# cloneofsimo/vqgan-training

Measured on AMD Instinct MI355X. Metric: images/sec full train step (enc+dec+LPIPS+disc+bwd), 256x256 f=8, higher is better.
Workload: dtype mixed like the reference: encoder+LPIPS+discriminator fp16 operands (TF32's 10-bit mantissa) / fp32 accumulate, decoder bf16

## Files before the change

### vqgan-training_amd/csrc/conv_small.hip

```cpp
#include "vq_common.h"

struct SmallConvParams {
  VqConvDesc d;
  const vq_bf16* x;
  const vq_bf16* w;
  const float* bias;
  const vq_bf16* relu_mask;
  vq_bf16* y;
  int M, HoWo, Kp;
  float alpha;
  const float* alpha_dev;
};

template <int DT, int FC>
__global__ __launch_bounds__(256) void conv3x3_c8_kernel(const SmallConvParams p) {
  const int lane = threadIdx.x & 63;
  const int fr = lane & 31, fh = lane >> 5;
  const int wave_global = blockIdx.x * 4 + (threadIdx.x >> 6);
  const int nwaves = gridDim.x * 4;

  s16x8 wf[FC][5];
#pragma unroll
  for (int a = 0; a < FC; ++a)
#pragma unroll
    for (int kk = 0; kk < 5; ++kk) {
      int row = a * 32 + fr;
      if (row >= p.d.Cout) row = p.d.Cout - 1;
      wf[a][kk] = *(const s16x8*)(p.w + (int64_t)row * p.Kp + kk * 16 + fh * 8);
    }
  typedef Store<DT> St;
  const float alpha = p.alpha_dev ? p.alpha * *p.alpha_dev : p.alpha;
  constexpr int CP = FC * 32, SPR = CP / 8;
  __shared__ __attribute__((aligned(16))) vq_bf16 slabs[4 * 32 * CP];
  vq_bf16* slab = slabs + (threadIdx.x >> 6) * 32 * CP;
  float bv[FC][4][4];
#pragma unroll
  for (int a = 0; a < FC; ++a)
#pragma unroll
    for (int q = 0; q < 4; ++q)
#pragma unroll
      for (int e = 0; e < 4; ++e) {
        const int co = a * 32 + q * 8 + fh * 4 + e;
        bv[a][q][e] = (p.bias && co < p.d.Cout_w) ? p.bias[co] : 0.f;
      }
  const int ngroups = (p.M + 31) >> 5;
  for (int g = wave_global; g < ngroups; g += nwaves) {
    const int m = g * 32 + fr;
    const bool live = m < p.M;
    const int mm = live ? m : p.M - 1;
    const int n = mm / p.HoWo, rem = mm - n * p.HoWo;
    const int oy = rem / p.d.Wo, ox = rem - oy * p.d.Wo;
    s16x8 bf[5];
#pragma unroll
    for (int kk = 0; kk < 5; ++kk) {
      const int tap = 2 * kk + fh;
      const int r = tap / 3, s = tap - r * 3;
      const int iy = oy + r - 1, ix = ox + s - 1;
      const bool ok = live && tap < 9 && (unsigned)iy < (unsigned)p.d.H && (unsigned)ix < (unsigned)p.d.W;
      s16x8 z;
#pragma unroll
      for (int e = 0; e < 8; ++e) z[e] = 0;
      bf[kk] = ok ? *(const s16x8*)(p.x + ((int64_t)(n * p.d.H + iy) * p.d.W + ix) * 8) : z;
    }
    f32x16 acc[FC];
#pragma unroll
    for (int a = 0; a < FC; ++a)
#pragma unroll
      for (int e = 0; e < 16; ++e) acc[a][e] = 0.f;
#pragma unroll
    for (int kk = 0; kk < 5; ++kk)
#pragma unroll
      for (int a = 0; a < FC; ++a) acc[a] = mfma16<DT>(wf[a][kk], bf[kk], acc[a]);
#pragma unroll
    for (int a = 0; a < FC; ++a)
#pragma unroll
      for (int q = 0; q < 4; ++q) {
        const int co = a * 32 + q * 8 + fh * 4;
        float v[4];
#pragma unroll
        for (int e = 0; e < 4; ++e) {
          v[e] = acc[a][q * 4 + e] * alpha + bv[a][q][e];
          if (p.d.relu) v[e] = v[e] > 0.f ? v[e] : 0.f;
        }
        St::store4(slab, fr * CP + ((((co >> 3) + fr) % SPR) << 3) + (co & 4), v);
      }
    vq_wave_sync();
    const int64_t m0 = (int64_t)g * 32;
#pragma unroll
    for (int it = 0; it < (32 * SPR) / 64; ++it) {
      const int i = it * 64 + lane, p_l = i / SPR, sl = i % SPR;
      if (m0 + p_l >= p.M || sl * 8 >= p.d.Cout) continue;
      float v[8];
      St::load8(slab, p_l * CP + (((sl + p_l) % SPR) << 3), v);
      const int64_t off = (m0 + p_l) * p.d.Cout + sl * 8;
      if (p.relu_mask) {
        float mv[8];
        St::load8(p.relu_mask, off, mv);
#pragma unroll
        for (int e = 0; e < 8; ++e) v[e] = mv[e] > 0.f ? v[e] : 0.f;
      }
      St::store8(p.y, off, v);
    }
    vq_wave_sync();
  }
}

bool vq_conv_c8_shape(const VqConvDesc* d) {
  return d->subpix == 0 && (d->dtype == VQ_BF16 || d->dtype == VQ_F16) && d->split == 1 && d->Cin == 8 && d->R == 3 && d->S == 3 && d->stride == 1 && d->dil_in == 1 &&
         d->up == 1 && d->pad_t == 1 && d->pad_l == 1 && d->Cout <= 128 && d->Ho == d->H && d->Wo == d->W;
}
int vq_launch_conv_c8(const VqConvDesc* d, const void* x, const void* w_packed, const float* bias, const void* residual,
                      const void* relu_mask, void* y, float alpha, const float* alpha_dev, hipStream_t stream) {
  if (!vq_conv_c8_shape(d) || residual != nullptr) return 1;
  SmallConvParams p;
  p.d = *d; p.x = (const vq_bf16*)x; p.w = (const vq_bf16*)w_packed; p.bias = bias; p.relu_mask = (const vq_bf16*)relu_mask;
  p.y = (vq_bf16*)y;
  p.M = d->N * d->Ho * d->Wo; p.HoWo = d->Ho * d->Wo;
  p.Kp = vq_round_up(9 * 8, 64);
  p.alpha = alpha; p.alpha_dev = alpha_dev;
  const int ngroups = (p.M + 31) / 32;
  int blocks = (ngroups + 3) / 4;
  if (blocks > 2048) blocks = 2048;
  const int fc = (d->Cout + 31) / 32;
#define VQ_C8(DTv) do { \
    if (fc == 1) hipLaunchKernelGGL((conv3x3_c8_kernel<DTv, 1>), dim3(blocks), dim3(256), 0, stream, p); \
    else if (fc == 2) hipLaunchKernelGGL((conv3x3_c8_kernel<DTv, 2>), dim3(blocks), dim3(256), 0, stream, p); \
    else if (fc == 3) hipLaunchKernelGGL((conv3x3_c8_kernel<DTv, 3>), dim3(blocks), dim3(256), 0, stream, p); \
    else hipLaunchKernelGGL((conv3x3_c8_kernel<DTv, 4>), dim3(blocks), dim3(256), 0, stream, p); } while (0)
  if (d->dtype == VQ_F16) VQ_C8(VQ_F16); else VQ_C8(VQ_BF16);
#undef VQ_C8
  VQ_CHECK_LAUNCH("vq_conv2d_fwd(c8)");
  return VQ_OK;
}

template <int FC>
__global__ __launch_bounds__(256) void conv3x3_c8_x2_kernel(const SmallConvParams p) {
  typedef Store<VQ_F16X2> St;
  const int lane = threadIdx.x & 63, wave = threadIdx.x >> 6;
  const int fr = lane & 31, fh = lane >> 5;
  const int wave_global = blockIdx.x * 4 + wave, nwaves = gridDim.x * 4;
  __shared__ __attribute__((aligned(16))) float slabs[4 * 32 * 32];
  float* slab = slabs + wave * 32 * 32;
  const float alpha = p.alpha_dev ? p.alpha * *p.alpha_dev : p.alpha;
  const int ngroups = (p.M + 31) >> 5, nitems = ngroups * FC;
  int a_cur = -1;
  s16x8 wh[5], wl[5];
  float bv[4][4];
  for (int t = wave_global; t < nitems; t += nwaves) {
    const int g = t / FC, a = t - g * FC;
    if (a != a_cur) {
      a_cur = a;
      int row = a * 32 + fr;
      if (row >= p.d.Cout) row = p.d.Cout - 1;
#pragma unroll
      for (int kk = 0; kk < 5; ++kk) {
        const vq_bf16* src = p.w + (int64_t)row * p.Kp + (2 * kk + fh) * 16;
        wh[kk] = *(const s16x8*)src;
        wl[kk] = *(const s16x8*)(src + 8);
      }
#pragma unroll
      for (int q = 0; q < 4; ++q)
#pragma unroll
        for (int e = 0; e < 4; ++e) {
          const int co = a * 32 + q * 8 + fh * 4 + e;
          bv[q][e] = (p.bias && co < p.d.Cout_w) ? p.bias[co] : 0.f;
        }
    }
    const int m = g * 32 + fr;
    const bool live = m < p.M;
    const int mm = live ? m : p.M - 1;
    const int n = mm / p.HoWo, rem = mm - n * p.HoWo;
    const int oy = rem / p.d.Wo, ox = rem - oy * p.d.Wo;
    s16x8 bh[5], bl[5];
#pragma unroll
    for (int kk = 0; kk < 5; ++kk) {
      const int tap = 2 * kk + fh;
      const int r = tap / 3, sx = tap - r * 3;
      const int iy = oy + r - 1, ix = ox + sx - 1;
      const bool ok = live && tap < 9 && (unsigned)iy < (unsigned)p.d.H && (unsigned)ix < (unsigned)p.d.W;
      s16x8 z;
#pragma unroll
      for (int e = 0; e < 8; ++e) z[e] = 0;
      const vq_bf16* src = p.x + ((int64_t)(n * p.d.H + iy) * p.d.W + ix) * 16;
      bh[kk] = ok ? *(const s16x8*)src : z;
      bl[kk] = ok ? *(const s16x8*)(src + 8) : z;
    }
    f32x16 acc;
#pragma unroll
    for (int e = 0; e < 16; ++e) acc[e] = 0.f;
#pragma unroll
    for (int kk = 0; kk < 5; ++kk) {
      acc = mfma_32x32x16_f16(wh[kk], bl[kk], acc);
      acc = mfma_32x32x16_f16(wl[kk], bh[kk], acc);
      acc = mfma_32x32x16_f16(wh[kk], bh[kk], acc);
    }
#pragma unroll
    for (int q = 0; q < 4; ++q) {
      vq_f4 v;
      float t4[4];
#pragma unroll
      for (int e = 0; e < 4; ++e) {
        t4[e] = acc[q * 4 + e] * alpha + bv[q][e];
        if (p.d.relu) t4[e] = t4[e] > 0.f ? t4[e] : 0.f;
      }
      v.x = t4[0]; v.y = t4[1]; v.z = t4[2]; v.w = t4[3];
      *(vq_f4*)(slab + fr * 32 + (((q * 2 + fh) ^ (fr & 7)) << 2)) = v;
    }
    vq_wave_sync();
    const int64_t m0 = (int64_t)g * 32;
#pragma unroll
    for (int it = 0; it < 2; ++it) {
      const int i = it * 64 + lane, p_l = i >> 2, sl = i & 3;
      const int co = a * 32 + sl * 8;
      const vq_f4 lo4 = *(const vq_f4*)(slab + p_l * 32 + (((2 * sl) ^ (p_l & 7)) << 2));
      const vq_f4 hi4 = *(const vq_f4*)(slab + p_l * 32 + (((2 * sl + 1) ^ (p_l & 7)) << 2));
      if (m0 + p_l >= p.M || co >= p.d.Cout) continue;
      float v[8] = {lo4.x, lo4.y, lo4.z, lo4.w, hi4.x, hi4.y, hi4.z, hi4.w};
      const int64_t off = (m0 + p_l) * p.d.Cout + co;
      if (p.relu_mask) {
        float mv[8];
        St::load8(p.relu_mask, off, mv);
#pragma unroll
        for (int e = 0; e < 8; ++e) v[e] = mv[e] > 0.f ? v[e] : 0.f;
      }
      St::store8(p.y, off, v);
    }
    vq_wave_sync();
  }
}
bool vq_conv_c8_x2_shape(const VqConvDesc* d) {
  return d->dtype == VQ_F16X2 && d->subpix == 0 && d->split == 1 && d->Cin == 16 && d->R == 3 && d->S == 3 && d->stride == 1 && d->dil_in == 1 &&
         d->up == 1 && d->pad_t == 1 && d->pad_l == 1 && d->Cout <= 128 && d->Ho == d->H && d->Wo == d->W;
}
int vq_launch_conv_c8_x2(const VqConvDesc* d, const void* x, const void* w_packed, const float* bias, const void* residual,
                         const void* relu_mask, void* y, float alpha, const float* alpha_dev, hipStream_t stream) {
  if (!vq_conv_c8_x2_shape(d) || residual != nullptr) return 1;
  SmallConvParams p;
  p.d = *d; p.x = (const vq_bf16*)x; p.w = (const vq_bf16*)w_packed; p.bias = bias; p.relu_mask = (const vq_bf16*)relu_mask;
  p.y = (vq_bf16*)y;
  p.M = d->N * d->Ho * d->Wo; p.HoWo = d->Ho * d->Wo;
  p.Kp = vq_round_up(9 * 16, 64);
  p.alpha = alpha; p.alpha_dev = alpha_dev;
  const int fc = (d->Cout + 31) / 32;
  const int nitems = ((p.M + 31) / 32) * fc;
  int blocks = (nitems + 3) / 4;
  if (blocks > 2048) blocks = 2048;
  blocks = (blocks + 2) / 3 * 3;
  if (fc == 1) hipLaunchKernelGGL((conv3x3_c8_x2_kernel<1>), dim3(blocks), dim3(256), 0, stream, p);
  else if (fc == 2) hipLaunchKernelGGL((conv3x3_c8_x2_kernel<2>), dim3(blocks), dim3(256), 0, stream, p);
  else if (fc == 3) hipLaunchKernelGGL((conv3x3_c8_x2_kernel<3>), dim3(blocks), dim3(256), 0, stream, p);
  else hipLaunchKernelGGL((conv3x3_c8_x2_kernel<4>), dim3(blocks), dim3(256), 0, stream, p);
  VQ_CHECK_LAUNCH("vq_conv2d_fwd(c8, VQ_F16X2)");
  return VQ_OK;
}

struct SmallWgradParams {
  const vq_bf16* narrow;
  const vq_bf16* wide;
  float* part;
  int H, W, C;
  int M, runs_per_block, nruns;
  int nstride, noff;
};

template <int DT, int BT>
__global__ __launch_bounds__(256) void wgrad_c8_kernel(const SmallWgradParams p) {
  constexpr int RB = BT * 2, SPR = RB / 16, RPP = 1024 / RB, NPC = (64 / RPP) / 4;
  constexpr int XROW = 72 * 8;
  __shared__ __attribute__((aligned(16))) vq_bf16 lds[2 * 3 * XROW + 64 + 2 * 64 * BT];
  vq_bf16* zs = lds + 2 * 3 * XROW;
  auto xs_of = [&](int b) -> vq_bf16* { return lds + b * 3 * XROW; };
  auto ys_of = [&](int b) -> vq_bf16* { return lds + 2 * 3 * XROW + 64 + b * 64 * BT; };
  auto seg_key = [](int row) -> int { return RB >= 256 ? (row & 3) : ((row >> 1) & 1); };

  const int tid = threadIdx.x, lane = tid & 63, wave = tid >> 6;
  const int W = p.W, H = p.H;
  constexpr int NCF = BT / 32;
  const int my_cf = wave;
  f32x16 acc[3];
#pragma unroll
  for (int a = 0; a < 3; ++a)
#pragma unroll
    for (int e = 0; e < 16; ++e) acc[a][e] = 0.f;

  if (tid < 32) ((unsigned*)zs)[tid] = (tid == 30) ? (unsigned)One16<DT>::BITS : 0u;
  const int gg = lane >> 4, tl = lane & 15;
  int a_off[3];
  bool a_zero[3];
#pragma unroll
  for (int f = 0; f < 3; ++f) {
    const int tap = 4 * f + 2 * (gg & 1) + ((tl & 3) >> 1);
    a_zero[f] = tap >= 9;
    const int r = tap / 3, s = tap - r * 3;
    a_off[f] = a_zero[f] ? ((tap == 9 && (tl & 1) == 0) ? 60 : 0) : (r * XROW + (8 * (gg >> 1) + (tl >> 2) + s) * 8 + (tl & 1) * 4);
  }
  const int b_row = 8 * (gg >> 1) + (tl >> 2);
  const int b_col = (gg & 1) * 16 + (tl & 3) * 4;

  const int lrow = lane / SPR, lp = lane % SPR;
  const int ct0 = (int)blockIdx.y * BT;
  const int run0 = blockIdx.x * p.runs_per_block;
  int nhere = p.nruns - run0;
  if (nhere > p.runs_per_block) nhere = p.runs_per_block;

  auto stage_wide = [&](int run, int b) {
    const int m0 = run * 64;
    vq_bf16* ys = ys_of(b);
#pragma unroll
    for (int i = 0; i < NPC; ++i) {
      const int row = (wave * NPC + i) * RPP + lrow;
      const int seg = (lp >> 2) ^ seg_key(row);
      const int lsl = ((seg << 2) | (lp & 3)) << 3;
      glds16(p.wide + (int64_t)(m0 + row) * p.C + ct0 + lsl, ys + (wave * NPC + i) * RPP * BT);
    }
  };
  auto load_narrow = [&](int run) -> vq_u4 {
    vq_u4 v; v.x = v.y = v.z = v.w = 0u;
    if (tid < 3 * 66) {
      const int m0 = run * 64;
      const int n = m0 / (H * W), rem = m0 - n * H * W;
      const int oy = rem / W, ox0 = rem - oy * W;
      const int r = tid / 66, j = tid - r * 66;
      const int iy = oy + r - 1, ix = ox0 - 1 + j;
      if ((unsigned)iy < (unsigned)H && (unsigned)ix < (unsigned)W)
        v = *(const vq_u4*)(p.narrow + ((int64_t)(n * H + iy) * W + ix) * p.nstride + p.noff);
    }
    return v;
  };
  auto store_narrow = [&](int b, vq_u4 v) {
    if (tid < 3 * 66) {
      const int r = tid / 66, j = tid - r * 66;
      *(vq_u4*)(xs_of(b) + r * XROW + j * 8) = v;
    }
  };

  if (nhere > 0) {
    stage_wide(run0, 0);
    store_narrow(0, load_narrow(run0));
  }
  for (int rr = 0; rr < nhere; ++rr) {
    const int b = rr & 1;
    __syncthreads();
    const bool more = rr + 1 < nhere;
    vq_u4 nv; nv.x = nv.y = nv.z = nv.w = 0u;
    if (more) {
      stage_wide(run0 + rr + 1, b ^ 1);
      nv = load_narrow(run0 + rr + 1);
    }
    if (my_cf < NCF) {
      const vq_bf16* xs = xs_of(b);
      const char* yb = (const char*)ys_of(b);
#pragma unroll
      for (int kk = 0; kk < 4; ++kk) {
        const int c = my_cf * 32 + b_col;
        const int seg = (c * 2) >> 6, within = (c * 2) & 63;
        const int r0 = kk * 16 + b_row, r1 = r0 + 4;
        s16x4 lo4 = lds_read_tr16_b64((const short*)(yb + r0 * RB + ((seg ^ seg_key(r0)) << 6) + within));
        s16x4 hi4 = lds_read_tr16_b64((const short*)(yb + r1 * RB + ((seg ^ seg_key(r1)) << 6) + within));
        s16x8 bfr;
        bfr[0] = lo4[0]; bfr[1] = lo4[1]; bfr[2] = lo4[2]; bfr[3] = lo4[3];
        bfr[4] = hi4[0]; bfr[5] = hi4[1]; bfr[6] = hi4[2]; bfr[7] = hi4[3];
#pragma unroll
        for (int f = 0; f < 3; ++f) {
          const vq_bf16* base = a_zero[f] ? zs + a_off[f] : xs + a_off[f] + kk * 16 * 8;
          const int step = a_zero[f] ? 0 : 4 * 8;
          s16x4 al = lds_read_tr16_b64((const short*)base);
          s16x4 ah = lds_read_tr16_b64((const short*)(base + step));
          s16x8 af;
          af[0] = al[0]; af[1] = al[1]; af[2] = al[2]; af[3] = al[3];
          af[4] = ah[0]; af[5] = ah[1]; af[6] = ah[2]; af[7] = ah[3];
          acc[f] = mfma16<DT>(af, bfr, acc[f]);
        }
      }
    }
    if (more) store_narrow(b ^ 1, nv);
  }
  if (my_cf < NCF) {
    float* out = p.part + (int64_t)blockIdx.x * 96 * p.C;
    const int fr = lane & 31, fh = lane >> 5;
    const int c = ct0 + my_cf * 32 + fr;
#pragma unroll
    for (int f = 0; f < 3; ++f)
#pragma unroll
      for (int e = 0; e < 16; ++e) {
        const int i = f * 32 + (e & 3) + 8 * (e >> 2) + 4 * fh;
        out[(int64_t)i * p.C + c] = acc[f][e];
      }
  }
}

__global__ void wgrad_c8_reduce_kernel(const float* __restrict__ part, int nblk, int C, int Cout_w, int Cin_w,
                                       int swapped, int accumulate, float alpha, float* __restrict__ dw, float* __restrict__ dbias) {
  const int total = Cout_w * Cin_w * 9, total_b = total + (dbias ? Cout_w : 0);
  const int t = blockIdx.x * blockDim.x + threadIdx.x;
  const int i = t >> 3, sub = t & 7;
  const bool live = i < total_b, is_bias = i >= total;
  const int ii = (live && !is_bias) ? i : 0;
  const int tap = ii % 9, ci = (ii / 9) % Cin_w, co = is_bias ? (live ? i - total : 0) : ii / (9 * Cin_w);
  const int row = is_bias ? 72 : (swapped ? (8 - tap) * 8 + co : tap * 8 + ci), col = (swapped && !is_bias) ? ci : co;
  float s = 0.f;
  for (int b = sub; b < nblk; b += 8) s += part[((int64_t)b * 96 + row) * C + col];
  s += __shfl_xor(s, 1); s += __shfl_xor(s, 2); s += __shfl_xor(s, 4);
  s *= alpha;
  if (live && sub == 0) {
    float* dst = is_bias ? dbias + co : dw + ((int64_t)co * Cin_w + ci) * 9 + tap;
    *dst = accumulate ? (*dst + s) : s;
  }
}

static int c8_wgrad_blocks(const VqConvDesc* d) {
  const int nruns = d->N * d->Ho * d->Wo / 64;
  return nruns < 512 ? nruns : 512;
}
static bool c8_common(const VqConvDesc* d) {
  return (d->dtype == VQ_BF16 || d->dtype == VQ_F16) && d->split == 1 && d->R == 3 && d->S == 3 && d->stride == 1 && d->dil_in == 1 && d->up == 1 &&
         d->pad_t == 1 && d->pad_l == 1 && d->Ho == d->H && d->Wo == d->W && d->Wo % 64 == 0;
}
static bool c8_wide_ok(int c) { return c == 64 || (c % 128 == 0 && c >= 128 && c <= 1024); }
static bool c8_swapped(const VqConvDesc* d) { return d->Cout == 8 && c8_wide_ok(d->Cin); }
bool vq_wgrad_c8_eligible(const VqConvDesc* d) {
  return c8_common(d) && ((d->Cin == 8 && c8_wide_ok(d->Cout)) || c8_swapped(d));
}
size_t vq_wgrad_c8_workspace(const VqConvDesc* d) {
  return (size_t)c8_wgrad_blocks(d) * 96 * (c8_swapped(d) ? d->Cin : d->Cout) * sizeof(float);
}

static int c8_wgrad_grid(const VqConvDesc* d, int C, SmallWgradParams& p, dim3& grid) {
  p.H = d->H; p.W = d->W; p.C = C;
  p.M = d->N * d->Ho * d->Wo;
  p.nruns = p.M / 64;
  const int nblk = c8_wgrad_blocks(d);
  p.runs_per_block = (p.nruns + nblk - 1) / nblk;
  const int used = (p.nruns + p.runs_per_block - 1) / p.runs_per_block;
  grid = dim3(used, C >= 128 ? C / 128 : 1);
  return used;
}
#define WGRAD_C8_ROWS(X) X(VQ_F16, 128) X(VQ_F16, 64) X(VQ_BF16, 128) X(VQ_BF16, 64)
static void launch_wgrad_c8_pass(int dtype, const SmallWgradParams& p, dim3 grid, hipStream_t stream) {
  const int dt = dtype == VQ_F16 ? VQ_F16 : VQ_BF16, bt = vq_wgrad_c8_tile(p.C);
#define X(DT, BT) if (dt == DT && bt == BT) hipLaunchKernelGGL((wgrad_c8_kernel<DT, BT>), grid, dim3(256), 0, stream, p);
  WGRAD_C8_ROWS(X)
#undef X
}

int vq_launch_wgrad_c8(const VqConvDesc* d, const void* x, const void* dy, float* dw, float* dbias, int* dbias_done,
                       int accumulate, float alpha, void* workspace, hipStream_t stream) {
  const bool sw = c8_swapped(d);
  SmallWgradParams p;
  p.narrow = (const vq_bf16*)(sw ? dy : x); p.wide = (const vq_bf16*)(sw ? x : dy); p.part = (float*)workspace;
  p.nstride = 8; p.noff = 0;
  dim3 grid;
  const int used = c8_wgrad_grid(d, sw ? d->Cin : d->Cout, p, grid);
  launch_wgrad_c8_pass(d->dtype, p, grid, stream);
  VQ_CHECK_LAUNCH("vq_conv2d_wgrad(c8)");
  float* db = sw ? nullptr : dbias;
  *dbias_done = db != nullptr;
  const int total = d->Cout_w * d->Cin_w * 9 + (db ? d->Cout_w : 0);
  hipLaunchKernelGGL(wgrad_c8_reduce_kernel, dim3((total * 8 + 255) / 256), dim3(256), 0, stream, (const float*)workspace, used,
                     p.C, d->Cout_w, d->Cin_w, sw ? 1 : 0, accumulate, alpha, dw, db);
  VQ_CHECK_LAUNCH("vq_conv2d_wgrad(c8 reduce)");
  return VQ_OK;
}


__global__ void wgrad_c8_reduce_x2_kernel(const float* __restrict__ part_h, const float* __restrict__ part_l, int nblk, int CV, int Cout_w,
                                          int Cin_w, int swapped, int accumulate, float alpha, float* __restrict__ dw, float* __restrict__ dbias) {
  const int total = Cout_w * Cin_w * 9, total_b = total + (dbias ? Cout_w : 0);
  const int t = blockIdx.x * blockDim.x + threadIdx.x;
  const int i = t >> 3, sub = t & 7;
  const bool live = i < total_b, is_bias = i >= total;
  const int ii = (live && !is_bias) ? i : 0;
  const int tap = ii % 9, ci = (ii / 9) % Cin_w, co = is_bias ? (live ? i - total : 0) : ii / (9 * Cin_w);
  const int row = is_bias ? 72 : (swapped ? (8 - tap) * 8 + co : tap * 8 + ci), wc = (swapped && !is_bias) ? ci : co;
  const int col = ((wc >> 3) << 4) + (wc & 7);
  float big = 0.f, small = 0.f;
  for (int b = sub; b < nblk; b += 8) {
    const float* ph = part_h + ((int64_t)b * 96 + row) * CV + col;
    big += ph[0];
    if (is_bias) small += ph[8];
    else { const float* pl = part_l + ((int64_t)b * 96 + row) * CV + col; small += (ph[8] + pl[0]) + pl[8]; }
  }
  big += __shfl_xor(big, 1); big += __shfl_xor(big, 2); big += __shfl_xor(big, 4);
  small += __shfl_xor(small, 1); small += __shfl_xor(small, 2); small += __shfl_xor(small, 4);
  const float r = (big + small) * alpha;
  if (live && sub == 0) {
    float* dst = is_bias ? dbias + co : dw + ((int64_t)co * Cin_w + ci) * 9 + tap;
    *dst = accumulate ? (*dst + r) : r;
  }
}
static bool c8_x2_swapped(const VqConvDesc* d) { return d->Cout == 8 && c8_wide_ok(2 * d->Cin); }
bool vq_wgrad_c8_x2_eligible(const VqConvDesc* d) {
  return d->dtype == VQ_F16X2 && d->split == 1 && d->R == 3 && d->S == 3 && d->stride == 1 && d->dil_in == 1 && d->up == 1 && d->pad_t == 1 &&
         d->pad_l == 1 && d->Ho == d->H && d->Wo == d->W && d->Wo % 64 == 0 && d->alpha_dev == nullptr &&
         ((d->Cin == 8 && c8_wide_ok(2 * d->Cout)) || c8_x2_swapped(d));
}
size_t vq_wgrad_c8_x2_workspace(const VqConvDesc* d) {
  return (size_t)2 * c8_wgrad_blocks(d) * 96 * 2 * (c8_x2_swapped(d) ? d->Cin : d->Cout) * sizeof(float);
}
int vq_launch_wgrad_c8_x2(const VqConvDesc* d, const void* x, const void* dy, float* dw, float* dbias, int* dbias_done, int accumulate,
                          float alpha, void* workspace, hipStream_t stream) {
  const bool sw = c8_x2_swapped(d);
  SmallWgradParams p;
  p.narrow = (const vq_bf16*)(sw ? dy : x); p.wide = (const vq_bf16*)(sw ? x : dy);
  p.nstride = 16;
  dim3 grid;
  const int used = c8_wgrad_grid(d, 2 * (sw ? d->Cin : d->Cout), p, grid);
  float* part_h = (float*)workspace;
  float* part_l = part_h + (size_t)c8_wgrad_blocks(d) * 96 * p.C;
  for (int pl = 0; pl < 2; ++pl) {
    p.noff = pl * 8; p.part = pl ? part_l : part_h;
    launch_wgrad_c8_pass(VQ_F16, p, grid, stream);
  }
  VQ_CHECK_LAUNCH("vq_conv2d_wgrad(c8, VQ_F16X2)");
  float* db = sw ? nullptr : dbias;
  *dbias_done = db != nullptr;
  const int total = d->Cout_w * d->Cin_w * 9 + (db ? d->Cout_w : 0);
  hipLaunchKernelGGL(wgrad_c8_reduce_x2_kernel, dim3((total * 8 + 255) / 256), dim3(256), 0, stream, (const float*)part_h, (const float*)part_l,
                     used, p.C, d->Cout_w, d->Cin_w, sw ? 1 : 0, accumulate, alpha, dw, db);
  VQ_CHECK_LAUNCH("vq_conv2d_wgrad(c8 reduce, VQ_F16X2)");
  return VQ_OK;
}
```

Baseline: 277.5.

## Software-pipeline tap loads in c8 conv kernel and size grid to residency

Restructures the Cin=8 3x3 conv kernel so each wave prefetches the next group's input taps while computing the current one. Out-of-bounds taps are loaded from a safe address and zeroed by bitmask instead of branching. A full-tile fast path drops bounds checks and prefetches the relu mask early. Bias moves to shared memory instead of registers, launch bounds now set occupancy per channel count, and the grid is capped at resident blocks rather than a fixed 2048. This adds register pressure and slightly more complex code for a kernel that is only a small part of the full train step.

New measurement: 278.4 (median of 6 runs). About the same (+0.3%).

```diff
diff --git a/vqgan-training_amd/csrc/conv_small.hip b/vqgan-training_amd/csrc/conv_small.hip
--- a/vqgan-training_amd/csrc/conv_small.hip
+++ b/vqgan-training_amd/csrc/conv_small.hip
@@ -12,8 +12,100 @@
   const float* alpha_dev;
 };
 
+__device__ __forceinline__ void c8_load_taps(const SmallConvParams& p, int g, int fr, int fh, s16x8 (&bf)[5], unsigned& dead) {
+  const int m = g * 32 + fr;
+  const bool live = m < p.M;
+  const int mm = live ? m : p.M - 1;
+  const int n = mm / p.HoWo, rem = mm - n * p.HoWo;
+  const int oy = rem / p.d.Wo, ox = rem - oy * p.d.Wo;
+  dead = 0u;
+#pragma unroll
+  for (int kk = 0; kk < 5; ++kk) {
+    const int tap = 2 * kk + fh;
+    const int r = tap / 3, s = tap - r * 3;
+    const int iy = oy + r - 1, ix = ox + s - 1;
+    const bool ok = live && tap < 9 && (unsigned)iy < (unsigned)p.d.H && (unsigned)ix < (unsigned)p.d.W;
+    if (!ok) dead |= 1u << kk;
+    bf[kk] = *(const s16x8*)(p.x + ((int64_t)(n * p.d.H + (ok ? iy : oy)) * p.d.W + (ok ? ix : ox)) * 8);
+  }
+}
+__device__ __forceinline__ void c8_zero_dead_taps(s16x8 (&bf)[5], unsigned dead) {
+#pragma unroll
+  for (int kk = 0; kk < 5; ++kk) {
+    const unsigned keep = ((dead >> kk) & 1u) ? 0u : ~0u;
+    vq_u32x4 q = __builtin_bit_cast(vq_u32x4, bf[kk]);
+    q.x &= keep; q.y &= keep; q.z &= keep; q.w &= keep;
+    bf[kk] = __builtin_bit_cast(s16x8, q);
+  }
+}
+
+template <int DT, int FC, bool WHOLE>
+__device__ __forceinline__ void c8_trip(const SmallConvParams& p, int g, const s16x8 (&wf)[FC][5], const s16x8 (&bf)[5], float alpha,
+                                        vq_bf16* slab, const float* bias_s, int lane) {
+  typedef Store<DT> St;
+  constexpr int CP = FC * 32, SPR = CP / 8, IT = (32 * SPR) / 64;
+  const int fr = lane & 31, fh = lane >> 5;
+  const int64_t m0 = (int64_t)g * 32;
+  f32x16 acc[FC];
+#pragma unroll
+  for (int a = 0; a < FC; ++a)
+#pragma unroll
+    for (int e = 0; e < 16; ++e) acc[a][e] = 0.f;
+#pragma unroll
+  for (int kk = 0; kk < 5; ++kk)
+#pragma unroll
+    for (int a = 0; a < FC; ++a) acc[a] = mfma16<DT>(wf[a][kk], bf[kk], acc[a]);
+  typename St::Raw mk[IT];
+  if constexpr (WHOLE) {
+    if (p.relu_mask) {
+#pragma unroll
+      for (int it = 0; it < IT; ++it) {
+        const int i = it * 64 + lane;
+        St::load8_raw(mk[it], p.relu_mask, (m0 + i / SPR) * CP + (i % SPR) * 8);
+      }
+    }
+  }
+#pragma unroll
+  for (int a = 0; a < FC; ++a)
+#pragma unroll
+    for (int q = 0; q < 4; ++q) {
+      const int co = a * 32 + q * 8 + fh * 4;
+      const vq_f4 b4 = *(const vq_f4*)(bias_s + co);
+      const float bq[4] = {b4.x, b4.y, b4.z, b4.w};
+      float v[4];
+#pragma unroll
+      for (int e = 0; e < 4; ++e) {
+        v[e] = acc[a][q * 4 + e] * alpha + bq[e];
+        if (p.d.relu) v[e] = v[e] > 0.f ? v[e] : 0.f;
+      }
+      St::store4(slab, fr * CP + ((((co >> 3) + fr) % SPR) << 3) + (co & 4), v);
+    }
+  vq_wave_sync();
+#pragma unroll
+  for (int it = 0; it < IT; ++it) {
+    const int i = it * 64 + lane, p_l = i / SPR, sl = i % SPR;
+    if constexpr (!WHOLE) {
+      if (m0 + p_l >= p.M || sl * 8 >= p.d.Cout) continue;
+    }
+    float v[8];
+    St::load8(slab, p_l * CP + (((sl + p_l) % SPR) << 3), v);
+    const int64_t off = (m0 + p_l) * p.d.Cout + sl * 8;
+    if (p.relu_mask) {
+      float mv[8];
+      if constexpr (WHOLE) St::unpack8(mk[it], mv);
+      else St::load8(p.relu_mask, off, mv);
+#pragma unroll
+      for (int e = 0; e < 8; ++e) v[e] = mv[e] > 0.f ? v[e] : 0.f;
+    }
+    St::store8(p.y, off, v);
+  }
+  vq_wave_sync();
+}
+
+constexpr int c8_blocks_per_cu(int fc) { return fc >= 3 ? 2 : (fc == 2 ? 3 : 4); }
+
 template <int DT, int FC>
-__global__ __launch_bounds__(256) void conv3x3_c8_kernel(const SmallConvParams p) {
+__global__ __launch_bounds__(256, c8_blocks_per_cu(FC)) void conv3x3_c8_kernel(const SmallConvParams p) {
   const int lane = threadIdx.x & 63;
   const int fr = lane & 31, fh = lane >> 5;
   const int wave_global = blockIdx.x * 4 + (threadIdx.x >> 6);
@@ -28,80 +120,40 @@
       if (row >= p.d.Cout) row = p.d.Cout - 1;
       wf[a][kk] = *(const s16x8*)(p.w + (int64_t)row * p.Kp + kk * 16 + fh * 8);
     }
-  typedef Store<DT> St;
   const float alpha = p.alpha_dev ? p.alpha * *p.alpha_dev : p.alpha;
-  constexpr int CP = FC * 32, SPR = CP / 8;
-  __shared__ __attribute__((aligned(16))) vq_bf16 slabs[4 * 32 * CP];
+  constexpr int CP = FC * 32;
+  __shared__ __attribute__((aligned(16))) vq_bf16 slabs[4 * 32 * CP + 2 * CP];
   vq_bf16* slab = slabs + (threadIdx.x >> 6) * 32 * CP;
-  float bv[FC][4][4];
-#pragma unroll
-  for (int a = 0; a < FC; ++a)
-#pragma unroll
-    for (int q = 0; q < 4; ++q)
-#pragma unroll
-      for (int e = 0; e < 4; ++e) {
-        const int co = a * 32 + q * 8 + fh * 4 + e;
-        bv[a][q][e] = (p.bias && co < p.d.Cout_w) ? p.bias[co] : 0.f;
-      }
+  float* bias_s = (float*)(slabs + 4 * 32 * CP);
+  if ((int)threadIdx.x < CP) bias_s[threadIdx.x] = (p.bias && (int)threadIdx.x < p.d.Cout_w) ? p.bias[threadIdx.x] : 0.f;
+  __syncthreads();
   const int ngroups = (p.M + 31) >> 5;
-  for (int g = wave_global; g < ngroups; g += nwaves) {
-    const int m = g * 32 + fr;
-    const bool live = m < p.M;
-    const int mm = live ? m : p.M - 1;
-    const int n = mm / p.HoWo, rem = mm - n * p.HoWo;
-    const int oy = rem / p.d.Wo, ox = rem - oy * p.d.Wo;
+  const int nwhole = p.d.Cout == CP ? (p.M >> 5) : 0;
+  int g = wave_global;
+  if (g < nwhole) {
+    s16x8 bn[5];
+    unsigned dead_n;
+    c8_load_taps(p, g, fr, fh, bn, dead_n);
+    wait_vmcnt<0>();
+    for (;;) {
+      s16x8 bf[5];
+#pragma unroll
+      for (int kk = 0; kk < 5; ++kk) bf[kk] = bn[kk];
+      const unsigned dead = dead_n;
+      const int gn = g + nwaves;
+      c8_load_taps(p, gn < nwhole ? gn : nwhole - 1, fr, fh, bn, dead_n);
+      c8_zero_dead_taps(bf, dead);
+      c8_trip<DT, FC, true>(p, g, wf, bf, alpha, slab, bias_s, lane);
+      g = gn;
+      if (gn >= nwhole) break;
+    }
+  }
+  for (; g < ngroups; g += nwaves) {
     s16x8 bf[5];
-#pragma unroll
-    for (int kk = 0; kk < 5; ++kk) {
-      const int tap = 2 * kk + fh;
-      const int r = tap / 3, s = tap - r * 3;
-      const int iy = oy + r - 1, ix = ox + s - 1;
-      const bool ok = live && tap < 9 && (unsigned)iy < (unsigned)p.d.H && (unsigned)ix < (unsigned)p.d.W;
-      s16x8 z;
-#pragma unroll
-      for (int e = 0; e < 8; ++e) z[e] = 0;
-      bf[kk] = ok ? *(const s16x8*)(p.x + ((int64_t)(n * p.d.H + iy) * p.d.W + ix) * 8) : z;
-    }
-    f32x16 acc[FC];
-#pragma unroll
-    for (int a = 0; a < FC; ++a)
-#pragma unroll
-      for (int e = 0; e < 16; ++e) acc[a][e] = 0.f;
-#pragma unroll
-    for (int kk = 0; kk < 5; ++kk)
-#pragma unroll
-      for (int a = 0; a < FC; ++a) acc[a] = mfma16<DT>(wf[a][kk], bf[kk], acc[a]);
-#pragma unroll
-    for (int a = 0; a < FC; ++a)
-#pragma unroll
-      for (int q = 0; q < 4; ++q) {
-        const int co = a * 32 + q * 8 + fh * 4;
-        float v[4];
-#pragma unroll
-        for (int e = 0; e < 4; ++e) {
-          v[e] = acc[a][q * 4 + e] * alpha + bv[a][q][e];
-          if (p.d.relu) v[e] = v[e] > 0.f ? v[e] : 0.f;
-        }
-        St::store4(slab, fr * CP + ((((co >> 3) + fr) % SPR) << 3) + (co & 4), v);
-      }
-    vq_wave_sync();
-    const int64_t m0 = (int64_t)g * 32;
-#pragma unroll
-    for (int it = 0; it < (32 * SPR) / 64; ++it) {
-      const int i = it * 64 + lane, p_l = i / SPR, sl = i % SPR;
-      if (m0 + p_l >= p.M || sl * 8 >= p.d.Cout) continue;
-      float v[8];
-      St::load8(slab, p_l * CP + (((sl + p_l) % SPR) << 3), v);
-      const int64_t off = (m0 + p_l) * p.d.Cout + sl * 8;
-      if (p.relu_mask) {
-        float mv[8];
-        St::load8(p.relu_mask, off, mv);
-#pragma unroll
-        for (int e = 0; e < 8; ++e) v[e] = mv[e] > 0.f ? v[e] : 0.f;
-      }
-      St::store8(p.y, off, v);
-    }
-    vq_wave_sync();
+    unsigned dead;
+    c8_load_taps(p, g, fr, fh, bf, dead);
+    c8_zero_dead_taps(bf, dead);
+    c8_trip<DT, FC, false>(p, g, wf, bf, alpha, slab, bias_s, lane);
   }
 }
 
@@ -119,9 +171,13 @@
   p.Kp = vq_round_up(9 * 8, 64);
   p.alpha = alpha; p.alpha_dev = alpha_dev;
   const int ngroups = (p.M + 31) / 32;
+  const int fc = (d->Cout + 31) / 32;
   int blocks = (ngroups + 3) / 4;
-  if (blocks > 2048) blocks = 2048;
-  const int fc = (d->Cout + 31) / 32;
+  const int resident = 256 * c8_blocks_per_cu(fc);
+  if (blocks > resident) blocks = resident;
+#ifdef VQ_ABLATION_KERNELS
+  if (((d->kernel_hint >> 4) & 0xfffff) == 2 && blocks > 2) blocks = 2;
+#endif
 #define VQ_C8(DTv) do { \
     if (fc == 1) hipLaunchKernelGGL((conv3x3_c8_kernel<DTv, 1>), dim3(blocks), dim3(256), 0, stream, p); \
     else if (fc == 2) hipLaunchKernelGGL((conv3x3_c8_kernel<DTv, 2>), dim3(blocks), dim3(256), 0, stream, p); \
```
